# mlpc-ucsd/BDM

Measured on AMD Instinct MI355X. Metric: sampled shapes/sec (4096 pts, 1000 DDPM steps), higher is better.
Workload: dtype f32

## Files before the change

bdm_amd/csrc/sparse_conv_os.hip:

```cpp
#include <stdlib.h>

#include "../../include/bdm_hip.h"
#include "common.h"

using namespace bdm;

#include "sparse_h2_common.h"

#define OS_PAIRS 14

typedef __attribute__((ext_vector_type(4))) float f32x4a;
typedef float f32x4v_t __attribute__((ext_vector_type(4)));


#define TILE_REC 16
#define DILH_XCAP 1376

static void sconv_dil_geometry(int r, int half_tile, int *tile, int *xcap, int *tiles_max) {
  if (half_tile > 0) {
    *tile = half_tile;
    *xcap = DILH_XCAP;
  } else {
    *tile = r == 32 ? 512 : (r == 16 ? 256 : 128);
    *xcap = 3 * r * r;
// ... 222 lines not shown

extern "C" int bdm_voxel_dilate_slices(int r, int tile) {
  int tl, xcap, tiles_max;
  sconv_dil_geometry(r, half_tile_ok(r, tile) ? tile : 0, &tl, &xcap, &tiles_max);
  return tiles_max;
}

static int voxel_dilate_launch(int b, int r, int n_dil_max, const int *src, int thr, int *dil_list, int *dil_index, int *plane_start,
                               int *tile_start, int *class_count, int half_tile, void *stream) {
  BDM_REQUIRE(b >= 0 && (r == 8 || r == 16 || r == 32) && n_dil_max >= 1 && src && dil_list && dil_index && plane_start && tile_start,
              "voxel_dilate: bad arguments (r in {8, 16, 32})");
  BDM_REQUIRE(half_tile_ok(r, half_tile), "voxel_dilate: tile %d unsupported (0 = full tiles; 64 / 128 / 256: EXPERIMENTAL=1 builds)", half_tile);
  if (b == 0) return BDM_OK;
  int tile, xcap, tiles_max;
  sconv_dil_geometry(r, half_tile, &tile, &xcap, &tiles_max);
  BDM_REQUIRE(cdiv(r * r * r, tile) <= 1024, "voxel_dilate: more flat tiles than threads");
  const size_t smem = sizeof(unsigned) * (4 * (size_t)r * r + 1 + 32 + 2 * (r + 2));
  hipLaunchKernelGGL(vox_dilate_kernel, dim3(b), dim3(1024), smem, (hipStream_t)stream, r, n_dil_max, tile, xcap, tiles_max,
                     half_tile > 0 ? 1 : 0, src, thr, dil_list, dil_index, plane_start, tile_start, class_count);
  return launch_status("voxel_dilate");
}

extern "C" int bdm_voxel_dilate(int b, int r, int n_dil_max, const int *cnt, int *dil_list, int *dil_index, int *plane_start,
                                int *tile_start, int tile, void *stream) {
  return voxel_dilate_launch(b, r, n_dil_max, cnt, 0, dil_list, dil_index, plane_start, tile_start, nullptr, tile, stream);
}

extern "C" int bdm_voxel_dilate_again(int b, int r, int n_dil_max, const int *dil_index_in, int *dil_list, int *dil_index,
                                      int *plane_start, int *tile_start, int *class_count, int tile, void *stream) {
  BDM_REQUIRE(class_count != nullptr, "voxel_dilate_again: class_count is NULL");
  return voxel_dilate_launch(b, r, n_dil_max, dil_index_in, -1, dil_list, dil_index, plane_start, tile_start, class_count, tile, stream);
}

#ifdef DIL_TIMING
__device__ long long *g_dil_ts = nullptr;
extern "C" int bdm_debug_dil_timestamps(long long *buf) { return hipMemcpyToSymbol(HIP_SYMBOL(g_dil_ts), &buf, sizeof(buf)) == hipSuccess ? 0 : 1; }
#define DIL_STAMP(i) do { if (g_dil_ts && tid == 0) { g_dil_ts[(size_t)item * 8 + (i)] = wall_clock64();                                  \
    if ((i) == 0) g_dil_ts[(size_t)item * 8 + 7] = (long long)__builtin_amdgcn_s_getreg(63492) | ((long long)__builtin_amdgcn_s_getreg(63508) << 32); } } while (0)
#else
#define DIL_STAMP(i)
#endif

template <int MT, int NT, int NW, int R, bool H2IN>
__global__ __launch_bounds__(NW * 64) void sconv_dil_kernel(
    int C8, int Cout, int n_max, int n_dil_max, int xcap, const float4 *__restrict__ xr, const float *__restrict__ amax,
    const float4 *__restrict__ xconst, float x_inv_scale,
    const int *__restrict__ occ_index, const int *__restrict__ dil_list, const int *__restrict__ dil_index,
    const int *__restrict__ tile_start, const float4 *__restrict__ wq,
    const float *__restrict__ inv_scale, const float *__restrict__ bias, float *__restrict__ y, int compact, int gn_cg,
    double *__restrict__ gn_partial, int gn_slices, int nb_shapes, int ncb, int tiles_max, int *__restrict__ work_counter) {
  extern __shared__ __align__(16) float4 smem4[];
  constexpr int BM = 16 * MT, TILE = NT * NW * 16;
  constexpr int R2 = R * R, R3 = R2 * R;
  constexpr int NT_ = NW * 64;
  constexpr int WV = OS_PAIRS * 2 * 2 * BM, WI = (WV + NT_ - 1) / NT_;
  constexpr int NQ = OS_PAIRS / 2;
  constexpr int PF = MT * NT >= 16 ? 1 : 2;
  constexpr int NBLK = NT * NW, NB = MT * 4 * 2;
  float4 *Ws = smem4;
  float4 *Xs = smem4 + WV;
  const int XS = xcap + 128;
  __shared__ int s_item;
  __shared__ float s_osc[64], s_obi[64];

  const int tid0 = threadIdx.x;
  const int G = gn_partial != nullptr ? Cout / gn_cg : 0, S = gn_slices;
  const int items = tiles_max * ncb * nb_shapes;
  for (;;) {
    int tid = tid0;
    asm volatile("" : "+v"(tid));
    const int lane = tid & 63, wave = tid >> 6, l16 = lane & 15, kg = lane >> 4;
    __syncthreads();
    if (tid == 0) s_item = atomicAdd(work_counter, 1);
    __syncthreads();
    const int item = s_item;
    if (item >= items) break;
    const int bi = item % nb_shapes, m0 = ((item / nb_shapes) % ncb) * BM, tile = item / (nb_shapes * ncb);
  const int4 *te = reinterpret_cast<const int4 *>(tile_start + ((size_t)bi * tiles_max + tile) * TILE_REC);
  const int4 ta = te[0], tb = te[1];
  const int j0 = ta.x, jn = ta.y, v_first = ta.z, v_end = ta.w, k_lo = tb.x;
  const int tiles_live = tb.w, tile_x0 = tb.z >> 8, tile_x1 = tb.z & 255;
// ... 66 lines not shown
  auto store_chunk = [&](int c8) {
#pragma unroll
    for (int u = 0; u < PF; ++u)
      if (tid + u * NT_ < nrows) {
        const float4 p = make_float4(xa[u][0][0], xa[u][0][1], xa[u][0][2], xa[u][0][3]);
        const float4 q = make_float4(xa[u][1][0], xa[u][1][1], xa[u][1][2], xa[u][1][3]);
        put(tid + u * NT_, p, q);
      }
    for (int row0 = tid + PF * NT_; row0 < nrows; row0 += 2 * NT_) {
      const int row1 = row0 + NT_, rc1 = min(row1, nrows - 1);
      float4 a0, a1, b0, b1;
      if (H2IN) {
        const float4 *src = xr + (((size_t)bi * C8 + c8) * 2) * n_max + k_lo;
        a0 = src[row0]; a1 = src[n_max + row0]; b0 = src[rc1]; b1 = src[n_max + rc1];
      } else {
        const float4 *src = xb + ((size_t)c8 * n_max + k_lo) * 2;
        a0 = src[2 * row0]; a1 = src[2 * row0 + 1]; b0 = src[2 * rc1]; b1 = src[2 * rc1 + 1];
      }
      put(row0, a0, a1);
      if (row1 < nrows) put(row1, b0, b1);
    }
    if (H2IN && tid < 128) *reinterpret_cast<f32x4v *>(&Xs[(tid >> 6) * XS + xcap + 64 + (tid & 63)]) = cr;
#pragma unroll
    for (int i = 0; i < WI; ++i) {
      const int e = tid + i * NT_;
      if (e < WV) *reinterpret_cast<f32x4v *>(&Ws[e]) = wr[i];
    }
  };

  if (!nothing) load_chunk(0);

  int rec[NT][NQ];
  unsigned amask = 0u;
  {
    const int pl0 = max(tile_x0 - 1, 0), pl1 = min(tile_x1 + 1, R - 1), n_oi = (pl1 - pl0 + 1) * R2;
    const bool staged = !nothing && n_oi * (int)sizeof(int) <= 2 * XS * (int)sizeof(float4);
    int *s_oi = reinterpret_cast<int *>(Xs);
    const int *oi = occ_index + (size_t)bi * R3;
    int vq[NT];
#pragma unroll
    for (int q = 0; q < NT; ++q) {
      const int j = j0 + (q * NW + wave) * 16 + l16;
      vq[q] = j < jn ? dl[j] : -1;
    }
    if (staged) {
      const int4 *src = reinterpret_cast<const int4 *>(oi + pl0 * R2);
      for (int e = tid; e < n_oi / 4; e += NT_) reinterpret_cast<int4 *>(s_oi)[e] = src[e];
      __syncthreads();
    }
#pragma unroll
    for (int q = 0; q < NT; ++q) {
      const int v = vq[q];
      const int vx = v / R2, vy = (v / R) % R, vz = v % R;
#pragma unroll
      for (int Q = 0; Q < NQ; ++Q) {
        const int t = 4 * Q + kg;
        int k = -1;
        bool inside = false;
        if (v >= 0 && t < 27) {
          const int gx = vx + t / 9 - 1, gy = vy + (t / 3) % 3 - 1, gz = vz + t % 3 - 1;
          inside = gx >= 0 && gx < R && gy >= 0 && gy < R && gz >= 0 && gz < R;
          if (inside) k = staged ? s_oi[((gx - pl0) * R + gy) * R + gz] : oi[(gx * R + gy) * R + gz];
        }
        const bool here = k >= k_lo && k - k_lo < nrows;
        const bool live = here || (H2IN && inside);
        if (__ballot(live) != 0ull) amask |= 1u << (Q * NT + q);
        rec[q][Q] = here ? k - k_lo : ((H2IN && inside) ? xcap + 64 + lane : xcap + lane);
// ... 435 lines not shown
#pragma unroll
        for (int j = 0; j < NBLK; ++j) a += red[j * NB + e];
        red2[e] = a;
      }
      __syncthreads();
      const int ngt = BM / gn_cg;
      if (tid < ngt && m0 + tid * gn_cg < Cout) {
        double a = 0.0, qq = 0.0;
        const int nb4 = gn_cg / 4;
        for (int j = 0; j < nb4; ++j) {
          a += (double)red2[(tid * nb4 + j) * 2 + 0];
          qq += (double)red2[(tid * nb4 + j) * 2 + 1];
        }
        const double nfill = H2IN ? 0.0 : (double)((v_end - v_first) - (jn - j0));
        for (int c = 0; c < gn_cg; ++c) {
          const double bv = bias ? (double)bias[m0 + tid * gn_cg + c] : 0.0;
          a += nfill * bv;
          qq += nfill * bv * bv;
        }
        double *dst = gn_partial + (((size_t)bi * G + m0 / gn_cg + tid) * S + tile) * 2;
        dst[0] = a;
        dst[1] = qq;
      }
    }
    DIL_STAMP(6);
  }
}

#endif

static int sconv_dil_launch(bool h2in, int b, int cin, int cout, int r, int n_max, int n_dil_max, const void *xr, const float *amax,
                            const void *xconst, float x_inv_scale, const int *in_index, const int *dil_list, const int *dil_index,
                            const int *tile_start, const void *packed_w, const float *inv_scale, const float *bias, float *y,
                            int compact, int gn_cg, double *gn_partial, int *slices_out, int half_tile, int *work_counter,
                            void *stream) {
  BDM_REQUIRE(b >= 0 && cin >= 1 && cout >= 1 && n_max >= 1 && n_dil_max >= 1 && xr && (h2in ? xconst != nullptr : amax != nullptr) &&
                  in_index && dil_list && dil_index && tile_start && inv_scale && y && work_counter,
              "sparse_conv_dil: bad arguments");
  if (r != 8 && r != 16 && r != 32) {
    set_error("sparse_conv_dil: resolution %d unsupported (8, 16, 32)", r);
    return BDM_ERR_UNSUPPORTED;
  }
  BDM_REQUIRE(half_tile_ok(r, half_tile), "sparse_conv_dil: tile %d unsupported (0 = full tiles; 64 / 128 / 256: EXPERIMENTAL=1 builds)", half_tile);
  if (b == 0) return BDM_OK;
  const int c8 = (cin + 7) / 8;
  const int mi = cout > 32 ? 2 : 1;
  int tile, xcap, tiles;
  sconv_dil_geometry(r, half_tile, &tile, &xcap, &tiles);
  const int bm = 32 * mi, nblk = tile / 16, nb = (bm / 16) * 8, ncb = cdiv(cout, bm);
  size_t smem = half_tile ? 16 * (2 * ((size_t)xcap + 128))
                          : 16 * ((size_t)OS_PAIRS * 4 * bm + 2 * ((size_t)xcap + 128));
  const size_t smem_out = sizeof(float) * ((size_t)(nblk + 1) * nb + (compact ? 0 : (size_t)bm * tile));
  if (smem_out > smem) smem = smem_out;
  BDM_REQUIRE(!half_tile || smem + 1024 <= 81920, "sparse_conv_dil: the half-tile form needs two workgroups per CU (%zu bytes of LDS)", smem);
  static int cus[16] = {0};
  int dev = 0;
  (void)hipGetDevice(&dev);
  if (dev < 0 || dev >= 16 || cus[dev] == 0) {
    hipDeviceProp_t prop;
    const int n = hipGetDeviceProperties(&prop, dev) == hipSuccess ? prop.multiProcessorCount : 256;
    if (dev >= 0 && dev < 16) cus[dev] = n > 0 ? n : 256;
  }
  const int ncu = ((dev >= 0 && dev < 16) ? cus[dev] : 256) * (half_tile ? 2 : 1);
  const long long items = (long long)tiles * ncb * b;
  dim3 grid((unsigned)(items < ncu ? items : ncu));
  hipStream_t s = (hipStream_t)stream;
  const int slices = h2in ? tiles + 27 : tiles;
  if (gn_partial != nullptr) {
    BDM_REQUIRE(gn_cg >= 4 && (gn_cg & (gn_cg - 1)) == 0 && bm % gn_cg == 0 && cout % gn_cg == 0,
                "sparse_conv_dil: GroupNorm statistics need a power-of-two channels-per-group dividing %d (got cg=%d)", bm, gn_cg);
    if (slices_out) *slices_out = slices;
  }
#define DIL_LAUNCH_(MT, NT, NW, R, H)                                                                                      \
  do {                                                                                                                     \
    BDM_ALLOW_LDS((sconv_dil_kernel<MT, NT, NW, R, H>), smem);                                                             \
    hipLaunchKernelGGL((sconv_dil_kernel<MT, NT, NW, R, H>), grid, dim3(NW * 64), smem, s, c8, cout, n_max, n_dil_max,     \
                       xcap, (const float4 *)xr, amax, (const float4 *)xconst, x_inv_scale, in_index, dil_list, dil_index, \
                       tile_start, (const float4 *)packed_w, inv_scale, bias, y, compact, gn_cg, gn_partial, slices, b,    \
                       ncb, tiles, work_counter);                                                                          \
  } while (0)
#define DIL_LAUNCH(MT, NT, NW, R) do { if (h2in) DIL_LAUNCH_(MT, NT, NW, R, true); else DIL_LAUNCH_(MT, NT, NW, R, false); } while (0)
#define DILH_LAUNCH_(MT, NT, R, H)                                                                                         \
  do {                                                                                                                     \
    BDM_ALLOW_LDS((sconv_dilh_kernel<MT, NT, R, H>), smem);                                                                \
    hipLaunchKernelGGL((sconv_dilh_kernel<MT, NT, R, H>), grid, dim3(256), smem, s, c8, cout, n_max, n_dil_max,            \
                       (const float4 *)xr, amax, (const float4 *)xconst, x_inv_scale, in_index, dil_list, dil_index,       \
                       tile_start, (const float4 *)packed_w, inv_scale, bias, y, compact, gn_cg, gn_partial, slices, b,    \
                       ncb, tiles, work_counter);                                                                          \
  } while (0)
#define DILH_LAUNCH(MT, NT, R) do { if (h2in) DILH_LAUNCH_(MT, NT, R, true); else DILH_LAUNCH_(MT, NT, R, false); } while (0)
#define DILH_PICK(NT, R) do { if (mi == 2) DILH_LAUNCH(4, NT, R); else DILH_LAUNCH(2, NT, R); } while (0)
#ifdef BDM_EXPERIMENTAL
  if (half_tile) {
    const int nt = half_tile / 64;
    if (r == 32) { if (nt == 4) DILH_PICK(4, 32); else if (nt == 2) DILH_PICK(2, 32); else DILH_PICK(1, 32); }
    else if (r == 16) { if (nt == 4) DILH_PICK(4, 16); else if (nt == 2) DILH_PICK(2, 16); else DILH_PICK(1, 16); }
    else { if (nt == 2) DILH_PICK(2, 8); else DILH_PICK(1, 8); }
    return launch_status("sparse_conv_dil (half tiles)");
  }
#endif
  if (r == 32) { if (mi == 2) DIL_LAUNCH(4, 4, 8, 32); else DIL_LAUNCH(2, 4, 8, 32); }
  else if (r == 16) { if (mi == 2) DIL_LAUNCH(4, 2, 8, 16); else DIL_LAUNCH(2, 2, 8, 16); }
  else { if (mi == 2) DIL_LAUNCH(4, 1, 8, 8); else DIL_LAUNCH(2, 1, 8, 8); }
#undef DIL_LAUNCH
#undef DIL_LAUNCH_
#undef DILH_PICK
#undef DILH_LAUNCH
#undef DILH_LAUNCH_
  return launch_status("sparse_conv_dil");
}

extern "C" int bdm_sparse_conv_dil(int b, int cin, int cout, int r, int n_max, int n_dil_max, const void *xr, const float *amax,
                                   const int *occ_index, const int *dil_list, const int *dil_index, const int *tile_start,
                                   const void *packed_w, const float *inv_scale, const float *bias, float *y,
                                   int compact, int tile, int *work_counter, void *stream) {
  return sconv_dil_launch(false, b, cin, cout, r, n_max, n_dil_max, xr, amax, nullptr, 0.f, occ_index, dil_list, dil_index, tile_start,
                          packed_w, inv_scale, bias, y, compact, 0, nullptr, nullptr, tile, work_counter, stream);
}

extern "C" int bdm_sparse_conv_dil_gn(int b, int cin, int cout, int r, int n_max, int n_dil_max, const void *xr, const float *amax,
                                      const int *occ_index, const int *dil_list, const int *dil_index, const int *tile_start,
                                      const void *packed_w, const float *inv_scale, const float *bias,
                                      float *y, int compact, int groups, void *gn_partial, int *slices_out, int tile,
                                      int *work_counter, void *stream) {
  BDM_REQUIRE(groups >= 1 && cout % groups == 0 && gn_partial != nullptr && slices_out != nullptr, "sparse_conv_dil_gn: bad arguments");
  return sconv_dil_launch(false, b, cin, cout, r, n_max, n_dil_max, xr, amax, nullptr, 0.f, occ_index, dil_list, dil_index, tile_start,
                          packed_w, inv_scale, bias, y, compact, cout / groups, (double *)gn_partial, slices_out, tile, work_counter, stream);
}

extern "C" int bdm_sparse_conv_dil_h2_gn(int b, int cin, int cout, int r, int n_rows_max, int n_dil_max, const void *rows_h2,
                                         const void *xconst, float x_inv_scale, const int *in_index, const int *dil_list,
                                         const int *dil_index, const int *tile_start, const void *packed_w, const float *inv_scale,
                                         const float *bias, float *y, int groups, void *gn_partial, int *slices_out, int tile,
                                         int *work_counter, void *stream) {
  BDM_REQUIRE(groups >= 1 && cout % groups == 0 && gn_partial != nullptr && slices_out != nullptr && x_inv_scale > 0.f,
              "sparse_conv_dil_h2_gn: bad arguments");
  return sconv_dil_launch(true, b, cin, cout, r, n_rows_max, n_dil_max, rows_h2, nullptr, xconst, x_inv_scale, in_index, dil_list,
                          dil_index, tile_start, packed_w, inv_scale, bias, y, 1, cout / groups, (double *)gn_partial, slices_out, tile,
                          work_counter, stream);
}
```

bdm_amd/ops.py:

```python
import ctypes
import os

import torch

from . import _lib as L
from . import tape


def _bcl(t):
    if t.dtype != torch.float32:
        raise L.BdmHipError(f"expected float32, got {t.dtype}")
    B, C = t.shape[0], t.shape[1]
    if B * C > 0 and t.is_contiguous():
        l = t.numel() // (B * C)
        return t, B, C, l, C * l, l
    l = 1
    for s in t.shape[2:]:
        l *= s
    dense, exp = True, 1
    for d in range(t.dim() - 1, 1, -1):
        if t.shape[d] != 1 and t.stride(d) != exp:
            dense = False
        exp *= t.shape[d]
    if dense and C > 1 and t.stride(1) < l:
# ... 806 lines not shown
_amax_rings = {}
_static_epoch = 0
_static_epochs = 0


class static_step:

    def __enter__(self):
        global _static_epoch, _static_epochs
        _static_epochs += 1
        _static_epoch = _static_epochs

    def __exit__(self, *exc):
        global _static_epoch
        _static_epoch = 0
        return False


def _amax_slot(device):
    dev = torch.device(device)
    key = (str(device), torch._C._cuda_getCurrentRawStream(dev.index if dev.index is not None else torch._C._cuda_getDevice()))
    ring = _amax_rings.get(key)
    if ring is None or ring[1] >= ring[0].shape[0] or ring[2] != _static_epoch:
        ring = [torch.zeros(256, dtype=torch.float32, device=device), 0, _static_epoch]
        _amax_rings[key] = ring
    slot = ring[0][ring[1]:ring[1] + 1]
    ring[1] += 1
    return slot


class VoxelPlan:
    __slots__ = ("r", "n", "n_max", "coords", "norm_coords", "vox_coords", "ind", "cnt", "ws", "occ_index", "occ_list", "n_occ", "rowocc",
                 "ready", "stream", "dil_list", "dil_index", "plane_start", "tile_start", "n_dil_max",
                 "d2_list", "d2_index", "d2_tiles", "d2_class_count", "tile", "d2_tile")


_plan_cache = {}


def clear_plan_cache():
    _plan_cache.clear()


def voxel_plan(coords, r, eps=0.0, dilate=False):
    key = (coords.data_ptr(), coords._version, tuple(coords.shape), int(r))
    p = _plan_cache.get(key)
    if p is not None:
        ready = getattr(p, "ready", None)
        if ready is not None:
            if torch.cuda.current_stream(coords.device) != getattr(p, "stream", None):
                tape.wait_event(ready)
                p.ready = None
        return p
    lib = L.lib()
    B, _, n = coords.shape
    dev = coords.device
    r3 = r ** 3
    p = VoxelPlan()
    p.ready = None
    p.r, p.n, p.n_max = int(r), n, min(n, r3)
    p.coords = coords
    p.norm_coords, p.vox_coords = voxel_coords(coords, r, eps)
    p.ind = torch.empty(B, n, dtype=torch.int32, device=dev)
    p.cnt = torch.empty(B, r3, dtype=torch.int32, device=dev)
    p.ws = torch.empty(lib.bdm_voxelize_workspace_bytes(B, n, r), dtype=torch.uint8, device=dev)
    p.occ_index = torch.empty(B, r3, dtype=torch.int32, device=dev)
    p.occ_list = torch.empty(B, p.n_max, dtype=torch.int32, device=dev)
# ... 5 lines not shown
    p.dil_list = p.d2_list = None
    if dilate:
        plan_dilation(p)
        if dilate == 2:
            plan_dilation2(p)
    p.stream = torch.cuda.current_stream(dev) if coords.is_cuda else None
    _plan_cache[key] = p
    return p


def has_voxel_plan(coords, r):
    return (coords.data_ptr(), coords._version, tuple(coords.shape), int(r)) in _plan_cache


TILE_REC = 16
DIL_TILE = os.environ.get("BDM_DIL_TILE", "0")


def dil_tile(batch, n_points, r, second):
    if r not in (8, 16, 32) or DIL_TILE in ("0", "", "auto"):
        return 0
    if not L.has_experimental():
        raise L.BdmHipError(f"BDM_DIL_TILE={DIL_TILE}: the half-tile list convolution belongs to the experimental kernel families; "
                            "rebuild with `make -C bdm_amd/csrc EXPERIMENTAL=1`")
    return min(int(DIL_TILE), 128) if r == 8 else int(DIL_TILE)


DILATED_PLAN = True


def plan_dilation(p):
    if getattr(p, "dil_list", None) is not None:
        return p
    p.dil_list = p.dil_index = p.plane_start = p.tile_start = None
    p.n_dil_max = 0
    if not DILATED_PLAN or p.r not in (8, 16, 32):
        return p
    lib, B, r = L.lib(), p.cnt.shape[0], p.r
    dev = p.cnt.device
    p.n_dil_max = r ** 3
    p.tile = dil_tile(B, p.n, r, second=False)
    p.dil_list = torch.empty(B, p.n_dil_max, dtype=torch.int32, device=dev)
    p.dil_index = torch.empty(B, r ** 3, dtype=torch.int32, device=dev)
    p.plane_start = torch.empty(B, r + 2, dtype=torch.int32, device=dev)
    p.tile_start = torch.empty(B, lib.bdm_voxel_dilate_slices(r, p.tile), TILE_REC, dtype=torch.int32, device=dev)
    L.check(lib.bdm_voxel_dilate(B, r, p.n_dil_max, L.ptr(p.cnt), L.ptr(p.dil_list), L.ptr(p.dil_index), L.ptr(p.plane_start),
                                 L.ptr(p.tile_start), p.tile, L.stream()), "voxel_dilate")
    return p


def plan_dilation2(p):
    if getattr(p, "d2_list", None) is not None:
        return p
    plan_dilation(p)
    p.d2_list = p.d2_index = p.d2_tiles = p.d2_class_count = None
    if p.dil_list is None:
        return p
    lib, B, r = L.lib(), p.cnt.shape[0], p.r
    dev = p.cnt.device
    p.d2_tile = dil_tile(B, p.n, r, second=True)
    p.d2_list = torch.empty(B, p.n_dil_max, dtype=torch.int32, device=dev)
    p.d2_index = torch.empty(B, r ** 3, dtype=torch.int32, device=dev)
    ps = torch.empty(B, r + 2, dtype=torch.int32, device=dev)
    p.d2_tiles = torch.empty(B, lib.bdm_voxel_dilate_slices(r, p.d2_tile), TILE_REC, dtype=torch.int32, device=dev)
    p.d2_class_count = torch.empty(B, 27, dtype=torch.int32, device=dev)
    L.check(lib.bdm_voxel_dilate_again(B, r, p.n_dil_max, L.ptr(p.dil_index), L.ptr(p.d2_list), L.ptr(p.d2_index), L.ptr(ps),
                                       L.ptr(p.d2_tiles), L.ptr(p.d2_class_count), p.d2_tile, L.stream()), "voxel_dilate_again")
    return p


HOIST_CONDITIONING = os.environ.get("BDM_HOIST", "1") == "1"


def three_nn_search(points_coords, centers_coords):
    pc, cc = points_coords.contiguous(), centers_coords.contiguous()
    B, _, n = pc.shape
    m = cc.shape[2]
    idx = torch.empty(B, 3, n, dtype=torch.int32, device=pc.device)
    w = torch.empty(B, 3, n, dtype=torch.float32, device=pc.device)
    L.check(L.lib().bdm_three_nn_search(B, m, n, L.ptr(pc), L.ptr(cc), L.ptr(idx), L.ptr(w), L.stream()), "three_nn_search")
    return idx, w


def _fill_conditioning_map(feat, wf, out):
    xt = wf.t().contiguous()[None]
    for b in range(feat.shape[0]):
        pointwise_conv(xt, feat[b], out=out[b:b + 1])


def refresh_conditioning_maps(feat, maps):
    for key, ent in list(maps.items()):
        if len(ent) != 4:
            continue
        if ent[0] != ent[2]._version:
            del maps[key]
        else:
            _fill_conditioning_map(feat, ent[3]().contiguous(), ent[1])


class Conditioning:
# ... 189 lines not shown
        self.rows, self.plan, self.bias, self.channels = rows, plan, bias, channels

    is_cuda = property(lambda self: self.rows.is_cuda)
    device = property(lambda self: self.rows.device)

    def dense(self):
        B, r3, C = self.rows.shape[0], self.plan.r ** 3, self.channels
        out = self.bias.detach().view(1, C, 1).expand(B, C, r3).contiguous()
        idx = self.plan.dil_index.long()
        for b in range(B):
            v = torch.nonzero(idx[b] >= 0).squeeze(1)
            out[b, :, v] = self.rows[b, idx[b, v]].t()
        return out


def sparse_first_conv_os(features, plan, packed, bias, cout, gn_groups=None, compact=False):
    plan_dilation(plan)
    if plan.dil_list is None:
        raise L.BdmHipError(f"sparse_first_conv_os: resolution {plan.r} has no dilated plan (8, 16, 32)")
    f, B, C, n, bs_f, ld_f = _bcl(features)
    dev, lib, r = f.device, L.lib(), plan.r
    packed_w, inv_scale = packed
    xr = torch.empty(B, (C + 7) // 8, plan.n_max, 8, dtype=torch.float32, device=dev)
    slots = amax_slots(dev, B + 1)
    amax, counter = slots[:B], slots[B:]
    L.check(lib.bdm_sparse_voxel_features_f32(B, C, n, r, plan.n_max, L.ptr(f), bs_f, ld_f, L.ptr(plan.cnt), L.ptr(plan.ws),
                                              L.ptr(plan.occ_list), L.ptr(plan.n_occ), L.ptr(xr), L.ptr(amax), L.stream()),
            "sparse_voxel_features_f32")
    if compact:
        y = torch.empty(B, plan.n_dil_max, cout, dtype=torch.float32, device=dev)
        out = CompactGrid(y, plan, bias, cout)
    else:
        y = out = torch.empty(B, cout, r ** 3, dtype=torch.float32, device=dev)
    args = (B, C, cout, r, plan.n_max, plan.n_dil_max, L.ptr(xr), L.ptr(amax), L.ptr(plan.occ_index), L.ptr(plan.dil_list),
            L.ptr(plan.dil_index), L.ptr(plan.tile_start), L.ptr(packed_w), L.ptr(inv_scale), L.ptr(bias), L.ptr(y), 1 if compact else 0)
    if gn_groups:
        tiles = plan.tile_start.shape[1]
        partial = torch.empty(B, gn_groups, tiles, 2, dtype=torch.float64, device=dev)
        slices = ctypes.c_int(0)
        L.check(lib.bdm_sparse_conv_dil_gn(*args, int(gn_groups), L.ptr(partial), ctypes.byref(slices), plan.tile, L.ptr(counter), L.stream()),
                "sparse_conv_dil_gn")
        return out, (partial, tiles, int(gn_groups))
    L.check(lib.bdm_sparse_conv_dil(*args, plan.tile, L.ptr(counter), L.stream()), "sparse_conv_dil")
    return out


def to_h2_rows(x, plan, gn, stats, swish=True, saturated=None, bias=None):
    plan_dilation(plan)
    lib = L.lib()
    compact = isinstance(x, CompactGrid)
    src = x.rows if compact else x.contiguous()
    bias = x.bias if compact else bias
    B, C, V = src.shape[0], (x.channels if compact else src.shape[1]), plan.r ** 3
    dev = src.device
    s = float(h2_activation_scale(gn))
    C8 = (C + 7) // 8
    rows = torch.empty(B, C8, 2, plan.n_dil_max, 8, dtype=torch.float16, device=dev)
    const_h2 = torch.empty(B, C8, 2, 8, dtype=torch.float16, device=dev)
    const_f32 = torch.empty(B, C, dtype=torch.float32, device=dev)
    partial, slices, groups = stats
    L.check(lib.bdm_group_norm_to_h2_rows(B, C, V, groups, L.ptr(src), 0 if compact else 1, plan.n_dil_max, L.ptr(plan.dil_list),
                                          L.ptr(plan.tile_start), plan.tile_start.shape[1], L.ptr(bias), L.ptr(gn.weight), L.ptr(gn.bias),
                                          L.c_float(gn.eps), 1 if swish else 0, L.c_float(s), L.ptr(rows), L.ptr(const_h2), L.ptr(const_f32),
                                          L.ptr(partial), slices, L.ptr(saturated), L.stream()), "group_norm_to_h2_rows")
    return rows, const_h2, const_f32, 1.0 / s


def conv_class_pack(weight):
    cout, cin = weight.shape[:2]
    lib = L.lib()
    wsum = torch.empty(lib.bdm_conv3d_class_weight_elems(cout, cin), dtype=torch.float64, device=weight.device)
    L.check(lib.bdm_conv3d_class_weight_sums(cout, cin, L.ptr(weight.contiguous()), L.ptr(wsum), L.stream()), "conv3d_class_weight_sums")
    return wsum


def second_conv_rows(rows_h2, const_h2, const_f32, x_inv_scale, plan, packed, wsum, bias, cin, cout, groups=8):
    plan_dilation2(plan)
    lib, B, r = L.lib(), rows_h2.shape[0], plan.r
    dev = rows_h2.device
    packed_w, inv_scale = packed
    y = torch.empty(B, plan.n_dil_max, cout, dtype=torch.float32, device=dev)
    tiles = plan.d2_tiles.shape[1]
    partial = torch.empty(B, groups, tiles + 27, 2, dtype=torch.float64, device=dev)
    counter = amax_slots(dev, 1)
    slices = ctypes.c_int(0)
    L.check(lib.bdm_sparse_conv_dil_h2_gn(B, cin, cout, r, plan.n_dil_max, plan.n_dil_max, L.ptr(rows_h2), L.ptr(const_h2), L.c_float(x_inv_scale),
                                          L.ptr(plan.dil_index), L.ptr(plan.d2_list), L.ptr(plan.d2_index), L.ptr(plan.d2_tiles), L.ptr(packed_w),
                                          L.ptr(inv_scale), L.ptr(bias), L.ptr(y), int(groups), L.ptr(partial), ctypes.byref(slices), plan.d2_tile,
                                          L.ptr(counter), L.stream()), "sparse_conv_dil_h2_gn")
    assert slices.value == tiles + 27
    class_vals = torch.empty(B, 27, cout, dtype=torch.float32, device=dev)
    L.check(lib.bdm_conv3d_class_constants(B, cin, cout, L.ptr(wsum), L.ptr(bias), L.ptr(const_f32), L.ptr(plan.d2_class_count), L.ptr(class_vals),
                                           int(groups), L.ptr(partial), tiles + 27, tiles, L.stream()), "conv3d_class_constants")
    return y, class_vals, (partial, tiles + 27)


def se_gate_gn_rows(rows, class_vals, plan, stats, gn, w1, w2, pf=None, n_points=0):
    partial, slices = stats
    B, C = rows.shape[0], rows.shape[2]
    dev, lib = rows.device, L.lib()
    V = plan.r ** 3
    mean = torch.empty(B, C, dtype=torch.float32, device=dev)
    coef = torch.empty(B, C, 2, dtype=torch.float32, device=dev)
    gate = torch.empty(B, C, dtype=torch.float32, device=dev)
    part = torch.empty(lib.bdm_se_gate_gn_rows_workspace_elems(B, C), dtype=torch.float32, device=dev)
    args = (B, C, w1.shape[0], V, gn.num_groups, L.ptr(rows), plan.n_dil_max, L.ptr(plan.d2_tiles), plan.d2_tiles.shape[1], L.ptr(class_vals),
            L.ptr(plan.d2_class_count), L.ptr(partial), slices, L.ptr(gn.weight), L.ptr(gn.bias), L.c_float(gn.eps), L.ptr(w1), L.ptr(w2), L.ptr(part),
            L.ptr(mean), L.ptr(coef), L.ptr(gate))
    if pf is not None:
        (pp, ps, pg), pgn = pf
        pf_coef = torch.empty(B, C, 2, dtype=torch.float32, device=dev)
        L.check(lib.bdm_se_gate_gn_rows_pf(*args, L.ptr(pp), ps, pg, int(n_points), L.ptr(pgn.weight), L.ptr(pgn.bias), L.c_float(pgn.eps),
                                           L.ptr(pf_coef), L.stream()), "se_gate_gn_rows_pf")
        return gate, coef, pf_coef
    L.check(lib.bdm_se_gate_gn_rows(*args, L.stream()), "se_gate_gn_rows")
    return gate, coef


def devoxelize_gn_gate_add_rows(norm_coords, rows, class_vals, plan, coef, gate=None, add=None, add_coef=None):
    B, C = rows.shape[0], rows.shape[2]
    n = norm_coords.shape[2]
    out = torch.empty(B, C, n, dtype=torch.float32, device=rows.device)
# ... 85 lines not shown
```

include/bdm_hip.h:

```cpp
#ifndef BDM_HIP_H
#define BDM_HIP_H

#include <stddef.h>
#include <stdint.h>

#ifdef __cplusplus
extern "C" {
#endif

const char *bdm_last_error(void);
int bdm_abi_version(void);


int bdm_furthest_point_sampling(int b, int n, int m, const float *coords, int *indices,
                                float *centers_out, void *stream);

int bdm_gather_features_forward(int b, int c, int n, int m, const float *features,
                                const int *indices, float *out, void *stream);

int bdm_ball_query(int b, int n, int m, float radius, int u, const float *centers,
                   const float *points, int *neighbors, void *stream);

int bdm_grouping_forward(int b, int c, int n, int m, int u, const float *features,
                         const int *indices, float *out, void *stream);
// ... 234 lines not shown
#endif

size_t bdm_sparse_conv_h2_weight_elems(int cout, int cin);
int bdm_sparse_conv_pack_weights_h2(int cout, int cin, const float *w, void *packed, float *scale_ws,
                                    float *inv_scale, void *stream);
int bdm_sparse_split_h2(int b, int cin, int n_max, const void *xr, const float *amax, void *xh, void *stream);
int bdm_sparse_conv_gemm_h2(int b, int n_max, int cin, int cout, const void *xh, const float *amax, const void *packed_w,
                            const float *inv_scale, const int *n_occ, float *y, void *stream);
int bdm_sparse_conv_gemm_h2_cb(int b, int n_max, int cin, int cout, const void *xh, const float *amax, const void *packed_w,
                               const float *inv_scale, const int *n_occ, const float *col_bias, long long bs_cb, float *y, void *stream);

int bdm_voxel_dilate_slices(int r, int tile);
int bdm_voxel_dilate(int b, int r, int n_dil_max, const int *cnt, int *dil_list, int *dil_index, int *plane_start, int *tile_start,
                     int tile, void *stream);
int bdm_sparse_conv_dil(int b, int cin, int cout, int r, int n_max, int n_dil_max, const void *xr, const float *amax,
                        const int *occ_index, const int *dil_list, const int *dil_index, const int *tile_start,
                        const void *packed_w, const float *inv_scale, const float *bias, float *y, int compact, int tile,
                        int *work_counter, void *stream);
int bdm_sparse_conv_dil_gn(int b, int cin, int cout, int r, int n_max, int n_dil_max, const void *xr, const float *amax,
                           const int *occ_index, const int *dil_list, const int *dil_index, const int *tile_start,
                           const void *packed_w, const float *inv_scale, const float *bias, float *y, int compact, int groups,
                           void *gn_partial, int *slices_out, int tile, int *work_counter, void *stream);

int bdm_voxel_dilate_again(int b, int r, int n_dil_max, const int *dil_index_in, int *dil_list, int *dil_index, int *plane_start,
                           int *tile_start, int *class_count, int tile, void *stream);
int bdm_group_norm_to_h2_rows(int b, int c, int v, int groups, const float *x, int dense_in, int n_rows_max, const int *dil_list,
                              const int *tile_start, int tiles_max, const float *bias, const float *gamma, const float *beta,
                              float eps, int act, float act_scale, void *rows_h2, void *const_h2, float *const_f32,
                              const void *partial, int slices, unsigned int *saturated, void *stream);
int bdm_sparse_conv_dil_h2_gn(int b, int cin, int cout, int r, int n_rows_max, int n_dil_max, const void *rows_h2, const void *xconst,
                              float x_inv_scale, const int *in_index, const int *dil_list, const int *dil_index,
                              const int *tile_start, const void *packed_w, const float *inv_scale, const float *bias, float *y,
                              int groups, void *gn_partial, int *slices_out, int tile, int *work_counter, void *stream);
size_t bdm_conv3d_class_weight_elems(int cout, int cin);
int bdm_conv3d_class_weight_sums(int cout, int cin, const float *w, void *wsum, void *stream);
int bdm_conv3d_class_constants(int b, int cin, int cout, const void *wsum, const float *bias, const float *const_f32,
                               const int *class_count, float *class_vals, int groups, void *gn_partial, int slices, int slice0,
                               void *stream);
size_t bdm_se_gate_gn_rows_workspace_elems(int b, int c);
int bdm_se_gate_gn_rows(int b, int c, int hidden, int v, int groups, const float *rows, int n_rows_max, const int *tile_start,
                        int tiles_max, const float *class_vals, const int *class_count, const void *gn_partial, int slices,
                        const float *gamma, const float *beta, float eps, const float *w1, const float *w2, float *part_ws,
                        float *mean_ws, float *coef, float *gate, void *stream);
int bdm_se_gate_gn_rows_pf(int b, int c, int hidden, int v, int groups, const float *rows, int n_rows_max, const int *tile_start,
                           int tiles_max, const float *class_vals, const int *class_count, const void *gn_partial, int slices,
                           const float *gamma, const float *beta, float eps, const float *w1, const float *w2, float *part_ws,
                           float *mean_ws, float *coef, float *gate, const void *pf_partial, int pf_slices, int pf_groups, int pf_n,
                           const float *pf_gamma, const float *pf_beta, float pf_eps, float *pf_coef, void *stream);
int bdm_devoxelize_gn_gate_add_rows(int b, int c, int n, int r, const float *coords, const float *rows, int n_rows_max,
                                    const int *dil_index, const float *class_vals, const float *coef, const float *gate,
                                    const float *add, long long bs_a, int ld_a, float *out, long long bs_o, int ld_o, void *stream);
int bdm_devoxelize_gn_gate_add_rows_pf(int b, int c, int n, int r, const float *coords, const float *rows, int n_rows_max,
                                       const int *dil_index, const float *class_vals, const float *coef, const float *gate,
                                       const float *add, long long bs_a, int ld_a, const float *add_coef, float *out, long long bs_o,
                                       int ld_o, void *stream);


int bdm_ddpm_step(long long n, const float *x, const float *eps, const float *noise,
                  float sqrt_beta_prod, float sqrt_alpha_prod, float coef_x0, float coef_x,
                  float sigma, float *out, void *stream);
int bdm_ddpm_step_dev(long long n, const float *x, const float *eps, const float *noise, const float *coef,
                      float *out, void *stream);

int bdm_ddim_step(long long n, const float *x, const float *eps, const float *noise, float sqrt_beta_prod,
                  float sqrt_alpha_prod, float coef_x0, float coef_eps, float sigma, float *out, void *stream);

// ... 73 lines not shown
```

Before: 3.021.

## Precompute per-voxel neighbour row codes once per plan for dilated sparse conv

Adds a plan-time kernel that resolves each dilated voxel's 27 neighbours into 16-bit row offsets, with sentinels for zero and constant neighbours, and stores them per tile. The sparse-conv kernels can now read these packed records instead of staging occupancy-index planes in LDS and recomputing neighbour coordinates on every call. The records are reused across all diffusion steps that share the plan. It also adds an optional channel-block override, which currently defaults to automatic. The cost is an extra per-plan launch and extra global memory for the neighbour table.

```diff
diff --git a/bdm_amd/csrc/sparse_conv_os.hip b/bdm_amd/csrc/sparse_conv_os.hip
--- a/bdm_amd/csrc/sparse_conv_os.hip
+++ b/bdm_amd/csrc/sparse_conv_os.hip
@@ -278,6 +278,60 @@
   return voxel_dilate_launch(b, r, n_dil_max, dil_index_in, -1, dil_list, dil_index, plane_start, tile_start, class_count, tile, stream);
 }
 
+#define NBR_ZERO 0xffffu
+#define NBR_CONST 0xfffeu
+
+template <int R>
+__global__ __launch_bounds__(256) void vox_nbr_kernel(int n_dil_max, int tiles_max, int h2in, const int *__restrict__ in_index,
+                                                      const int *__restrict__ dil_list, const int *__restrict__ tile_start,
+                                                      uint4 *__restrict__ nbr) {
+  constexpr int R2 = R * R, R3 = R2 * R;
+  const int tile = blockIdx.x, bi = blockIdx.y;
+  const int4 *te = reinterpret_cast<const int4 *>(tile_start + ((size_t)bi * tiles_max + tile) * TILE_REC);
+  const int4 ta = te[0], tb = te[1];
+  const int j0 = ta.x, jn = ta.y, k_lo = tb.x, nrows = tb.y;
+  if (tile >= tb.w || jn <= j0) return;
+  const int *oi = in_index + (size_t)bi * R3;
+  const int *dl = dil_list + (size_t)bi * n_dil_max;
+  for (int e = threadIdx.x; e < (jn - j0) * 4; e += blockDim.x) {
+    const int j = j0 + (e >> 2), kg = e & 3;
+    const int v = dl[j];
+    const int vx = v / R2, vy = (v / R) % R, vz = v % R;
+    unsigned code[8];
+#pragma unroll
+    for (int Q = 0; Q < 8; ++Q) {
+      const int t = 4 * Q + kg;
+      unsigned c = NBR_ZERO;
+      if (t < 27) {
+        const int gx = vx + t / 9 - 1, gy = vy + (t / 3) % 3 - 1, gz = vz + t % 3 - 1;
+        const bool inside = gx >= 0 && gx < R && gy >= 0 && gy < R && gz >= 0 && gz < R;
+        const int k = inside ? oi[(gx * R + gy) * R + gz] : -1;
+        const bool here = k >= k_lo && k - k_lo < nrows;
+        c = here ? (unsigned)(k - k_lo) : ((h2in && inside) ? NBR_CONST : NBR_ZERO);
+      }
+      code[Q] = c;
+    }
+    nbr[((size_t)bi * n_dil_max + j) * 4 + kg] =
+        make_uint4(code[0] | (code[1] << 16), code[2] | (code[3] << 16), code[4] | (code[5] << 16), code[6] | (code[7] << 16));
+  }
+}
+
+extern "C" int bdm_voxel_dilate_nbr(int b, int r, int n_dil_max, const int *in_index, const int *dil_list, const int *tile_start,
+                                    int h2in, void *nbr, void *stream) {
+  BDM_REQUIRE(b >= 0 && (r == 8 || r == 16 || r == 32) && n_dil_max >= 1 && in_index && dil_list && tile_start && nbr,
+              "voxel_dilate_nbr: bad arguments (r in {8, 16, 32})");
+  if (b == 0) return BDM_OK;
+  int tile, xcap, tiles_max;
+  sconv_dil_geometry(r, 0, &tile, &xcap, &tiles_max);
+  static_assert(3 * 32 * 32 + 128 < (int)NBR_CONST, "row codes must stay below the sentinels");
+  const dim3 grid(tiles_max, b);
+  hipStream_t s = (hipStream_t)stream;
+  if (r == 32) hipLaunchKernelGGL(vox_nbr_kernel<32>, grid, dim3(256), 0, s, n_dil_max, tiles_max, h2in, in_index, dil_list, tile_start, (uint4 *)nbr);
+  else if (r == 16) hipLaunchKernelGGL(vox_nbr_kernel<16>, grid, dim3(256), 0, s, n_dil_max, tiles_max, h2in, in_index, dil_list, tile_start, (uint4 *)nbr);
+  else hipLaunchKernelGGL(vox_nbr_kernel<8>, grid, dim3(256), 0, s, n_dil_max, tiles_max, h2in, in_index, dil_list, tile_start, (uint4 *)nbr);
+  return launch_status("voxel_dilate_nbr");
+}
+
 #ifdef DIL_TIMING
 __device__ long long *g_dil_ts = nullptr;
 extern "C" int bdm_debug_dil_timestamps(long long *buf) { return hipMemcpyToSymbol(HIP_SYMBOL(g_dil_ts), &buf, sizeof(buf)) == hipSuccess ? 0 : 1; }
@@ -292,7 +346,7 @@
     int C8, int Cout, int n_max, int n_dil_max, int xcap, const float4 *__restrict__ xr, const float *__restrict__ amax,
     const float4 *__restrict__ xconst, float x_inv_scale,
     const int *__restrict__ occ_index, const int *__restrict__ dil_list, const int *__restrict__ dil_index,
-    const int *__restrict__ tile_start, const float4 *__restrict__ wq,
+    const int *__restrict__ tile_start, const uint4 *__restrict__ nbr, const float4 *__restrict__ wq,
     const float *__restrict__ inv_scale, const float *__restrict__ bias, float *__restrict__ y, int compact, int gn_cg,
     double *__restrict__ gn_partial, int gn_slices, int nb_shapes, int ncb, int tiles_max, int *__restrict__ work_counter) {
   extern __shared__ __align__(16) float4 smem4[];
@@ -425,7 +479,24 @@
 
   int rec[NT][NQ];
   unsigned amask = 0u;
-  {
+  if (nbr != nullptr) {
+    uint4 cw[NT];
+#pragma unroll
+    for (int q = 0; q < NT; ++q) {
+      const int j = j0 + (q * NW + wave) * 16 + l16;
+      cw[q] = j < jn ? nbr[((size_t)bi * n_dil_max + j) * 4 + kg] : make_uint4(~0u, ~0u, ~0u, ~0u);
+    }
+#pragma unroll
+    for (int q = 0; q < NT; ++q)
+#pragma unroll
+      for (int Q = 0; Q < NQ; ++Q) {
+        const unsigned w = Q < 2 ? cw[q].x : (Q < 4 ? cw[q].y : (Q < 6 ? cw[q].z : cw[q].w));
+        const unsigned c = (w >> (16 * (Q & 1))) & 0xffffu;
+        if (__ballot(c != NBR_ZERO) != 0ull) amask |= 1u << (Q * NT + q);
+        rec[q][Q] = c < NBR_CONST ? (int)c : (c == NBR_ZERO ? xcap + lane : xcap + 64 + lane);
+      }
+    amask = __builtin_amdgcn_readfirstlane(amask);
+  } else {
     const int pl0 = max(tile_x0 - 1, 0), pl1 = min(tile_x1 + 1, R - 1), n_oi = (pl1 - pl0 + 1) * R2;
     const bool staged = !nothing && n_oi * (int)sizeof(int) <= 2 * XS * (int)sizeof(float4);
     int *s_oi = reinterpret_cast<int *>(Xs);
@@ -927,11 +998,14 @@
 static int sconv_dil_launch(bool h2in, int b, int cin, int cout, int r, int n_max, int n_dil_max, const void *xr, const float *amax,
                             const void *xconst, float x_inv_scale, const int *in_index, const int *dil_list, const int *dil_index,
                             const int *tile_start, const void *packed_w, const float *inv_scale, const float *bias, float *y,
-                            int compact, int gn_cg, double *gn_partial, int *slices_out, int half_tile, int *work_counter,
-                            void *stream) {
+                            int compact, int gn_cg, double *gn_partial, int *slices_out, int half_tile, const void *nbr, int bm_req,
+                            int *work_counter, void *stream) {
   BDM_REQUIRE(b >= 0 && cin >= 1 && cout >= 1 && n_max >= 1 && n_dil_max >= 1 && xr && (h2in ? xconst != nullptr : amax != nullptr) &&
                   in_index && dil_list && dil_index && tile_start && inv_scale && y && work_counter,
               "sparse_conv_dil: bad arguments");
+  BDM_REQUIRE(bm_req == 0 || bm_req == 32 || bm_req == 64, "sparse_conv_dil: channel block %d unsupported (0 = by channel count, 32, 64)",
+              bm_req);
+  BDM_REQUIRE(nbr == nullptr || half_tile == 0, "sparse_conv_dil: neighbour records exist for full-tile plans only");
   if (r != 8 && r != 16 && r != 32) {
     set_error("sparse_conv_dil: resolution %d unsupported (8, 16, 32)", r);
     return BDM_ERR_UNSUPPORTED;
@@ -939,7 +1013,7 @@
   BDM_REQUIRE(half_tile_ok(r, half_tile), "sparse_conv_dil: tile %d unsupported (0 = full tiles; 64 / 128 / 256: EXPERIMENTAL=1 builds)", half_tile);
   if (b == 0) return BDM_OK;
   const int c8 = (cin + 7) / 8;
-  const int mi = cout > 32 ? 2 : 1;
+  const int mi = bm_req != 0 ? bm_req / 32 : (cout > 32 ? 2 : 1);
   int tile, xcap, tiles;
   sconv_dil_geometry(r, half_tile, &tile, &xcap, &tiles);
   const int bm = 32 * mi, nblk = tile / 16, nb = (bm / 16) * 8, ncb = cdiv(cout, bm);
@@ -971,8 +1045,8 @@
     BDM_ALLOW_LDS((sconv_dil_kernel<MT, NT, NW, R, H>), smem);                                                             \
     hipLaunchKernelGGL((sconv_dil_kernel<MT, NT, NW, R, H>), grid, dim3(NW * 64), smem, s, c8, cout, n_max, n_dil_max,     \
                        xcap, (const float4 *)xr, amax, (const float4 *)xconst, x_inv_scale, in_index, dil_list, dil_index, \
-                       tile_start, (const float4 *)packed_w, inv_scale, bias, y, compact, gn_cg, gn_partial, slices, b,    \
-                       ncb, tiles, work_counter);                                                                          \
+                       tile_start, (const uint4 *)nbr, (const float4 *)packed_w, inv_scale, bias, y, compact, gn_cg,       \
+                       gn_partial, slices, b, ncb, tiles, work_counter);                                                   \
   } while (0)
 #define DIL_LAUNCH(MT, NT, NW, R) do { if (h2in) DIL_LAUNCH_(MT, NT, NW, R, true); else DIL_LAUNCH_(MT, NT, NW, R, false); } while (0)
 #define DILH_LAUNCH_(MT, NT, R, H)                                                                                         \
@@ -1010,7 +1084,15 @@
                                    const void *packed_w, const float *inv_scale, const float *bias, float *y,
                                    int compact, int tile, int *work_counter, void *stream) {
   return sconv_dil_launch(false, b, cin, cout, r, n_max, n_dil_max, xr, amax, nullptr, 0.f, occ_index, dil_list, dil_index, tile_start,
-                          packed_w, inv_scale, bias, y, compact, 0, nullptr, nullptr, tile, work_counter, stream);
+                          packed_w, inv_scale, bias, y, compact, 0, nullptr, nullptr, tile, nullptr, 0, work_counter, stream);
+}
+
+extern "C" int bdm_sparse_conv_dil_nbr(int b, int cin, int cout, int r, int n_max, int n_dil_max, const void *xr, const float *amax,
+                                       const int *occ_index, const int *dil_list, const int *dil_index, const int *tile_start,
+                                       const void *nbr, const void *packed_w, const float *inv_scale, const float *bias, float *y,
+                                       int compact, int bm, int *work_counter, void *stream) {
+  return sconv_dil_launch(false, b, cin, cout, r, n_max, n_dil_max, xr, amax, nullptr, 0.f, occ_index, dil_list, dil_index, tile_start,
+                          packed_w, inv_scale, bias, y, compact, 0, nullptr, nullptr, 0, nbr, bm, work_counter, stream);
 }
 
 extern "C" int bdm_sparse_conv_dil_gn(int b, int cin, int cout, int r, int n_max, int n_dil_max, const void *xr, const float *amax,
@@ -1020,7 +1102,19 @@
                                       int *work_counter, void *stream) {
   BDM_REQUIRE(groups >= 1 && cout % groups == 0 && gn_partial != nullptr && slices_out != nullptr, "sparse_conv_dil_gn: bad arguments");
   return sconv_dil_launch(false, b, cin, cout, r, n_max, n_dil_max, xr, amax, nullptr, 0.f, occ_index, dil_list, dil_index, tile_start,
-                          packed_w, inv_scale, bias, y, compact, cout / groups, (double *)gn_partial, slices_out, tile, work_counter, stream);
+                          packed_w, inv_scale, bias, y, compact, cout / groups, (double *)gn_partial, slices_out, tile, nullptr, 0,
+                          work_counter, stream);
+}
+
+extern "C" int bdm_sparse_conv_dil_gn_nbr(int b, int cin, int cout, int r, int n_max, int n_dil_max, const void *xr, const float *amax,
+                                          const int *occ_index, const int *dil_list, const int *dil_index, const int *tile_start,
+                                          const void *nbr, const void *packed_w, const float *inv_scale, const float *bias, float *y,
+                                          int compact, int groups, void *gn_partial, int *slices_out, int bm, int *work_counter,
+                                          void *stream) {
+  BDM_REQUIRE(groups >= 1 && cout % groups == 0 && gn_partial != nullptr && slices_out != nullptr, "sparse_conv_dil_gn: bad arguments");
+  return sconv_dil_launch(false, b, cin, cout, r, n_max, n_dil_max, xr, amax, nullptr, 0.f, occ_index, dil_list, dil_index, tile_start,
+                          packed_w, inv_scale, bias, y, compact, cout / groups, (double *)gn_partial, slices_out, 0, nbr, bm,
+                          work_counter, stream);
 }
 
 extern "C" int bdm_sparse_conv_dil_h2_gn(int b, int cin, int cout, int r, int n_rows_max, int n_dil_max, const void *rows_h2,
@@ -1032,5 +1126,17 @@
               "sparse_conv_dil_h2_gn: bad arguments");
   return sconv_dil_launch(true, b, cin, cout, r, n_rows_max, n_dil_max, rows_h2, nullptr, xconst, x_inv_scale, in_index, dil_list,
                           dil_index, tile_start, packed_w, inv_scale, bias, y, 1, cout / groups, (double *)gn_partial, slices_out, tile,
-                          work_counter, stream);
-}
+                          nullptr, 0, work_counter, stream);
+}
+
+extern "C" int bdm_sparse_conv_dil_h2_gn_nbr(int b, int cin, int cout, int r, int n_rows_max, int n_dil_max, const void *rows_h2,
+                                             const void *xconst, float x_inv_scale, const int *in_index, const int *dil_list,
+                                             const int *dil_index, const int *tile_start, const void *nbr, const void *packed_w,
+                                             const float *inv_scale, const float *bias, float *y, int groups, void *gn_partial,
+                                             int *slices_out, int bm, int *work_counter, void *stream) {
+  BDM_REQUIRE(groups >= 1 && cout % groups == 0 && gn_partial != nullptr && slices_out != nullptr && x_inv_scale > 0.f,
+              "sparse_conv_dil_h2_gn: bad arguments");
+  return sconv_dil_launch(true, b, cin, cout, r, n_rows_max, n_dil_max, rows_h2, nullptr, xconst, x_inv_scale, in_index, dil_list,
+                          dil_index, tile_start, packed_w, inv_scale, bias, y, 1, cout / groups, (double *)gn_partial, slices_out, 0,
+                          nbr, bm, work_counter, stream);
+}
diff --git a/bdm_amd/ops.py b/bdm_amd/ops.py
--- a/bdm_amd/ops.py
+++ b/bdm_amd/ops.py
@@ -862,7 +862,7 @@
 class VoxelPlan:
     __slots__ = ("r", "n", "n_max", "coords", "norm_coords", "vox_coords", "ind", "cnt", "ws", "occ_index", "occ_list", "n_occ", "rowocc",
                  "ready", "stream", "dil_list", "dil_index", "plane_start", "tile_start", "n_dil_max",
-                 "d2_list", "d2_index", "d2_tiles", "d2_class_count", "tile", "d2_tile")
+                 "d2_list", "d2_index", "d2_tiles", "d2_class_count", "tile", "d2_tile", "nbr", "d2_nbr")
 
 
 _plan_cache = {}
@@ -934,7 +934,7 @@
 def plan_dilation(p):
     if getattr(p, "dil_list", None) is not None:
         return p
-    p.dil_list = p.dil_index = p.plane_start = p.tile_start = None
+    p.dil_list = p.dil_index = p.plane_start = p.tile_start = p.nbr = None
     p.n_dil_max = 0
     if not DILATED_PLAN or p.r not in (8, 16, 32):
         return p
@@ -948,14 +948,29 @@
     p.tile_start = torch.empty(B, lib.bdm_voxel_dilate_slices(r, p.tile), TILE_REC, dtype=torch.int32, device=dev)
     L.check(lib.bdm_voxel_dilate(B, r, p.n_dil_max, L.ptr(p.cnt), L.ptr(p.dil_list), L.ptr(p.dil_index), L.ptr(p.plane_start),
                                  L.ptr(p.tile_start), p.tile, L.stream()), "voxel_dilate")
+    p.nbr = plan_neighbours(p, p.occ_index, p.dil_list, p.tile_start, p.tile, h2in=0)
     return p
+
+
+def plan_neighbours(p, in_index, dil_list, tile_start, tile, h2in):
+    if tile != 0:
+        return None
+    B = in_index.shape[0]
+    nbr = torch.empty(B, p.n_dil_max, 4, 8, dtype=torch.int16, device=in_index.device)
+    L.check(L.lib().bdm_voxel_dilate_nbr(B, p.r, p.n_dil_max, L.ptr(in_index), L.ptr(dil_list), L.ptr(tile_start), h2in, L.ptr(nbr),
+                                         L.stream()), "voxel_dilate_nbr")
+    return nbr
+
+
+def dil_bm(cout, groups=None):
+    return 0
 
 
 def plan_dilation2(p):
     if getattr(p, "d2_list", None) is not None:
         return p
     plan_dilation(p)
-    p.d2_list = p.d2_index = p.d2_tiles = p.d2_class_count = None
+    p.d2_list = p.d2_index = p.d2_tiles = p.d2_class_count = p.d2_nbr = None
     if p.dil_list is None:
         return p
     lib, B, r = L.lib(), p.cnt.shape[0], p.r
@@ -968,6 +983,7 @@
     p.d2_class_count = torch.empty(B, 27, dtype=torch.int32, device=dev)
     L.check(lib.bdm_voxel_dilate_again(B, r, p.n_dil_max, L.ptr(p.dil_index), L.ptr(p.d2_list), L.ptr(p.d2_index), L.ptr(ps),
                                        L.ptr(p.d2_tiles), L.ptr(p.d2_class_count), p.d2_tile, L.stream()), "voxel_dilate_again")
+    p.d2_nbr = plan_neighbours(p, p.dil_index, p.d2_list, p.d2_tiles, p.d2_tile, h2in=1)
     return p
 
 
@@ -1223,16 +1239,29 @@
         out = CompactGrid(y, plan, bias, cout)
     else:
         y = out = torch.empty(B, cout, r ** 3, dtype=torch.float32, device=dev)
-    args = (B, C, cout, r, plan.n_max, plan.n_dil_max, L.ptr(xr), L.ptr(amax), L.ptr(plan.occ_index), L.ptr(plan.dil_list),
-            L.ptr(plan.dil_index), L.ptr(plan.tile_start), L.ptr(packed_w), L.ptr(inv_scale), L.ptr(bias), L.ptr(y), 1 if compact else 0)
+    nbr = getattr(plan, "nbr", None)
+    if nbr is None:
+        args = (B, C, cout, r, plan.n_max, plan.n_dil_max, L.ptr(xr), L.ptr(amax), L.ptr(plan.occ_index), L.ptr(plan.dil_list),
+                L.ptr(plan.dil_index), L.ptr(plan.tile_start), L.ptr(packed_w), L.ptr(inv_scale), L.ptr(bias), L.ptr(y), 1 if compact else 0)
+    else:
+        args = (B, C, cout, r, plan.n_max, plan.n_dil_max, L.ptr(xr), L.ptr(amax), L.ptr(plan.occ_index), L.ptr(plan.dil_list),
+                L.ptr(plan.dil_index), L.ptr(plan.tile_start), L.ptr(nbr), L.ptr(packed_w), L.ptr(inv_scale), L.ptr(bias), L.ptr(y),
+                1 if compact else 0)
     if gn_groups:
         tiles = plan.tile_start.shape[1]
         partial = torch.empty(B, gn_groups, tiles, 2, dtype=torch.float64, device=dev)
         slices = ctypes.c_int(0)
-        L.check(lib.bdm_sparse_conv_dil_gn(*args, int(gn_groups), L.ptr(partial), ctypes.byref(slices), plan.tile, L.ptr(counter), L.stream()),
-                "sparse_conv_dil_gn")
+        if nbr is None:
+            L.check(lib.bdm_sparse_conv_dil_gn(*args, int(gn_groups), L.ptr(partial), ctypes.byref(slices), plan.tile, L.ptr(counter),
+                                               L.stream()), "sparse_conv_dil_gn")
+        else:
+            L.check(lib.bdm_sparse_conv_dil_gn_nbr(*args, int(gn_groups), L.ptr(partial), ctypes.byref(slices), dil_bm(cout, gn_groups),
+                                                   L.ptr(counter), L.stream()), "sparse_conv_dil_gn_nbr")
         return out, (partial, tiles, int(gn_groups))
-    L.check(lib.bdm_sparse_conv_dil(*args, plan.tile, L.ptr(counter), L.stream()), "sparse_conv_dil")
+    if nbr is None:
+        L.check(lib.bdm_sparse_conv_dil(*args, plan.tile, L.ptr(counter), L.stream()), "sparse_conv_dil")
+    else:
+        L.check(lib.bdm_sparse_conv_dil_nbr(*args, dil_bm(cout), L.ptr(counter), L.stream()), "sparse_conv_dil_nbr")
     return out
 
 
@@ -1275,10 +1304,18 @@
     partial = torch.empty(B, groups, tiles + 27, 2, dtype=torch.float64, device=dev)
     counter = amax_slots(dev, 1)
     slices = ctypes.c_int(0)
-    L.check(lib.bdm_sparse_conv_dil_h2_gn(B, cin, cout, r, plan.n_dil_max, plan.n_dil_max, L.ptr(rows_h2), L.ptr(const_h2), L.c_float(x_inv_scale),
-                                          L.ptr(plan.dil_index), L.ptr(plan.d2_list), L.ptr(plan.d2_index), L.ptr(plan.d2_tiles), L.ptr(packed_w),
-                                          L.ptr(inv_scale), L.ptr(bias), L.ptr(y), int(groups), L.ptr(partial), ctypes.byref(slices), plan.d2_tile,
-                                          L.ptr(counter), L.stream()), "sparse_conv_dil_h2_gn")
+    nbr = getattr(plan, "d2_nbr", None)
+    if nbr is None:
+        L.check(lib.bdm_sparse_conv_dil_h2_gn(B, cin, cout, r, plan.n_dil_max, plan.n_dil_max, L.ptr(rows_h2), L.ptr(const_h2), L.c_float(x_inv_scale),
+                                              L.ptr(plan.dil_index), L.ptr(plan.d2_list), L.ptr(plan.d2_index), L.ptr(plan.d2_tiles), L.ptr(packed_w),
+                                              L.ptr(inv_scale), L.ptr(bias), L.ptr(y), int(groups), L.ptr(partial), ctypes.byref(slices), plan.d2_tile,
+                                              L.ptr(counter), L.stream()), "sparse_conv_dil_h2_gn")
+    else:
+        L.check(lib.bdm_sparse_conv_dil_h2_gn_nbr(B, cin, cout, r, plan.n_dil_max, plan.n_dil_max, L.ptr(rows_h2), L.ptr(const_h2),
+                                                  L.c_float(x_inv_scale), L.ptr(plan.dil_index), L.ptr(plan.d2_list), L.ptr(plan.d2_index),
+                                                  L.ptr(plan.d2_tiles), L.ptr(nbr), L.ptr(packed_w), L.ptr(inv_scale), L.ptr(bias), L.ptr(y),
+                                                  int(groups), L.ptr(partial), ctypes.byref(slices), dil_bm(cout, groups), L.ptr(counter),
+                                                  L.stream()), "sparse_conv_dil_h2_gn_nbr")
     assert slices.value == tiles + 27
     class_vals = torch.empty(B, 27, cout, dtype=torch.float32, device=dev)
     L.check(lib.bdm_conv3d_class_constants(B, cin, cout, L.ptr(wsum), L.ptr(bias), L.ptr(const_f32), L.ptr(plan.d2_class_count), L.ptr(class_vals),
diff --git a/include/bdm_hip.h b/include/bdm_hip.h
--- a/include/bdm_hip.h
+++ b/include/bdm_hip.h
@@ -290,6 +290,22 @@
                               float x_inv_scale, const int *in_index, const int *dil_list, const int *dil_index,
                               const int *tile_start, const void *packed_w, const float *inv_scale, const float *bias, float *y,
                               int groups, void *gn_partial, int *slices_out, int tile, int *work_counter, void *stream);
+
+int bdm_voxel_dilate_nbr(int b, int r, int n_dil_max, const int *in_index, const int *dil_list, const int *tile_start, int h2in,
+                         void *nbr, void *stream);
+int bdm_sparse_conv_dil_nbr(int b, int cin, int cout, int r, int n_max, int n_dil_max, const void *xr, const float *amax,
+                            const int *occ_index, const int *dil_list, const int *dil_index, const int *tile_start, const void *nbr,
+                            const void *packed_w, const float *inv_scale, const float *bias, float *y, int compact, int bm,
+                            int *work_counter, void *stream);
+int bdm_sparse_conv_dil_gn_nbr(int b, int cin, int cout, int r, int n_max, int n_dil_max, const void *xr, const float *amax,
+                               const int *occ_index, const int *dil_list, const int *dil_index, const int *tile_start, const void *nbr,
+                               const void *packed_w, const float *inv_scale, const float *bias, float *y, int compact, int groups,
+                               void *gn_partial, int *slices_out, int bm, int *work_counter, void *stream);
+int bdm_sparse_conv_dil_h2_gn_nbr(int b, int cin, int cout, int r, int n_rows_max, int n_dil_max, const void *rows_h2,
+                                  const void *xconst, float x_inv_scale, const int *in_index, const int *dil_list, const int *dil_index,
+                                  const int *tile_start, const void *nbr, const void *packed_w, const float *inv_scale,
+                                  const float *bias, float *y, int groups, void *gn_partial, int *slices_out, int bm,
+                                  int *work_counter, void *stream);
 size_t bdm_conv3d_class_weight_elems(int cout, int cin);
 int bdm_conv3d_class_weight_sums(int cout, int cin, const float *w, void *wsum, void *stream);
 int bdm_conv3d_class_constants(int b, int cin, int cout, const void *wsum, const float *bias, const float *const_f32,
```

New measurement: 3.012, median of 3. About the same (-0.3%).
